# iamwinter/UMPR

Measured on AMD Instinct MI355X. Metric: training samples/sec, higher is better.
Workload: dtype f32

## Files before the change

include/umpr_hip.h:

```cpp
#ifndef UMPR_HIP_H
#define UMPR_HIP_H
#include <stddef.h>
#include <stdint.h>

#ifdef __cplusplus
extern "C" {
#endif

const char* umpr_version(void);
const char* umpr_last_error(void);
int umpr_device_info(int dev, char* name, int name_len, int* compute_units, size_t* hbm_bytes);

int umpr_gemm_f32(const float* A, long lda, int transA, const float* B, long ldb, int transB, float* C, long ldc,
                  int M, int N, int K, const float* bias, int bias_mode, int act, int accumulate, float alpha,
                  float* ws, size_t ws_bytes, void* stream);

int umpr_set_gemm_bf16(int on);

int umpr_set_conv_inference(int on);

int umpr_set_conv_pool_follows(int on);

long umpr_debug_wino_fix_count(void);

int umpr_debug_conv3x3_plan(int pass, int N, int Cin, int Cout, int H, int W, int inference, size_t* ws_bytes, size_t* v_bytes);
int umpr_debug_conv_bf16_plan(int pass, int N, int Cin, int Cout, int H, int W, long* out);

int umpr_debug_wino_pool_fold(const float* y, const float* g_pooled, const float* w, const float* x, float* unpooled, float* dx,
                              float* dw, float* db, int N, int Cin, int Cout, int H, int W, int f4, int fold, float* ws,
                              size_t ws_bytes, void* stream);

size_t umpr_embed_gru_bidir_ws_bytes(int N, int L, int E);
int umpr_embed_gru_bidir_fwd(const int64_t* ids, const float* emb, int E,
                             const float* w_ih_f, const float* w_hh_f, const float* b_ih_f, const float* b_hh_f,
                             const float* w_ih_r, const float* w_hh_r, const float* b_ih_r, const float* b_hh_r,
                             const int32_t* lengths, const int32_t* order, const int32_t* dst_row, int N, int L,
                             float* out, float* saved, float* ws, size_t ws_bytes, void* stream);
int umpr_embed_gru_bidir_bwd(const int64_t* ids, const float* emb, int E,
                             const float* w_hh_f, const float* w_hh_r,
                             const int32_t* lengths, const int32_t* order, const int32_t* dst_row, int N, int L,
                             const float* dout, const float* out, const float* saved,
                             float* dw_ih_f, float* dw_hh_f, float* db_ih_f, float* db_hh_f,
                             float* dw_ih_r, float* dw_hh_r, float* db_ih_r, float* db_hh_r,
                             float* ws, size_t ws_bytes, void* stream);

// ... 303 lines not shown
```

umpr_amd/_lib.py:

```python
from __future__ import annotations

import ctypes
import os
import threading

import torch

_HERE = os.path.dirname(os.path.abspath(__file__))
LIB_PATH = os.path.join(_HERE, "libumpr_hip.so")

_T = {"p": ctypes.c_void_p, "i": ctypes.c_int, "l": ctypes.c_long, "z": ctypes.c_size_t, "f": ctypes.c_float,
      "d": ctypes.c_double, "u": ctypes.c_uint64}

SIGNATURES = {
    "umpr_version": ("", "s"),
    "umpr_last_error": ("", "s"),
    "umpr_device_info": ("ipipp", "i"),
    "umpr_gemm_f32": ("pliplipliiipiiifpzp", "i"),
    "umpr_embed_gru_bidir_ws_bytes": ("iii", "z"),
    "umpr_embed_gru_bidir_fwd": ("ppipppppppppppiipppzp", "i"),
    "umpr_embed_gru_bidir_bwd": ("ppipppppiippppppppppppzp", "i"),
    "umpr_embed_gru_bidir_bwd_acc": ("ppipppppiipppppppppppipzp", "i"),
    "umpr_embed_gru_bidir_bwd_dx": ("ppipppppiipppppppppppipppipzp", "i"),
    "umpr_embed_grad_chunk": ("", "i"),
# ... 98 lines not shown
    "umpr_grad_norm": ("ppidfppzpp", "i"),
    "umpr_adam_step_clip": ("ppppldddddld" "pp", "i"),
    "umpr_adam_step_dev_clip": ("pppplddd" "ppp", "i"),
    "umpr_adam_step_groups": ("ppppldddddld" "pp" "ppp" "ii" "p", "i"),
    "umpr_grad_accumulate": ("pppiip", "i"),
    "umpr_ema_update": ("pppidip", "i"),
    "umpr_arena_swap": ("pppip", "i"),
    "umpr_debug_poison_lds": ("pp", "i"),
    "umpr_set_gemm_bf16": ("i", "i"),
    "umpr_set_conv_inference": ("i", "i"),
    "umpr_set_conv_pool_follows": ("i", "i"),
    "umpr_debug_wino_fix_count": ("", "l"),
    "umpr_debug_conv3x3_plan": ("iiiiiiipp", "i"),
    "umpr_debug_conv_bf16_plan": ("iiiiiip", "i"),
    "umpr_debug_wino_pool_fold": ("pppppppp" "iiiiiii" "pzp", "i"),
    "umpr_profile_enable": ("i", "i"),
    "umpr_profile_reset": ("", "i"),
    "umpr_profile_read": ("ippp", "i"),
}


class UmprHipError(RuntimeError):
    pass


class _Tls(threading.local):
    gemm_b16 = False


TLS = _Tls()
# ... 73 lines not shown
```

umpr_amd/csrc/api.hip:

```cpp
#include <math.h>
#include <stdarg.h>
#include <stdlib.h>

#include <vector>

#include "../../include/umpr_hip.h"
#include "umpr_common.h"
#include "umpr_internal.h"

static thread_local char g_err[512] = "";
void umpr_set_error(const char* fmt, ...) {
  va_list ap;
  va_start(ap, fmt);
  vsnprintf(g_err, sizeof(g_err), fmt, ap);
  va_end(ap);
}

namespace {
const bool g_fc_small = umpr_env_on("UMPR_FC_SMALL");
struct ProfRec { hipEvent_t e0, e1; int family; double work; };
bool g_prof_on = false;
std::vector<ProfRec> g_prof;
std::vector<ProfRec> g_prof_pool;
double g_prof_ms[UMPR_K_COUNT] = {0}, g_prof_work[UMPR_K_COUNT] = {0};
// ... 122 lines not shown
  UMPR_REQUIRE(!dx || (f4 && w), "debug_wino_pool_fold: the data gradient runs on the 4x4 tile and needs the weights");
  UMPR_REQUIRE(!dw || (x && (!f4 || ((H_ % 4) == 0 && (W % 4) == 0))), "debug_wino_pool_fold: the weight gradient on the 4x4 tile has no edge tiles");
  hipStream_t s = S(stream);
  ConvHints h;
  const float* g = g_pooled;
  if (fold) { h.pooled_dy = true; h.pool_y = y; }
  else {
    if (int rc = umpr_maxpool2_bwd_relu_impl(y, g_pooled, unpooled, (long)N * Cout, H_, W, s)) return rc;
    g = unpooled;
  }
  if (dx)
    if (int rc = umpr_wino_conv3x3(g, w, 1, nullptr, nullptr, dx, N, Cin, Cout, H_, W, 0, ws, ws_bytes / sizeof(float), true, h, s)) return rc;
  if (dw)
    if (int rc = umpr_wino_wgrad(g, x, dw, db, N, Cin, Cout, H_, W, 0, ws, ws_bytes / sizeof(float), f4 != 0, h, s)) return rc;
  return 0;
}

constexpr size_t kSlabs = 256;
namespace {
struct GruWs {
  float *gx, *wslab, *bslab;
  float* kslab; size_t kslab_bytes;
  float *stacked, *rows;
  float *wst, *bst;
  size_t bytes;
};
GruWs gru_ws(float* base, int N, int L, int pitch) {
  Carve c(base, sizeof(float));
  const size_t tiles = umpr_gru_tiles(N);
  GruWs w;
// ... 1011 lines not shown
```

umpr_amd/csrc/umpr_internal.h:

```cpp
#pragma once
#include <hip/hip_runtime.h>
#include <stdint.h>

struct UmprGemm {
  const float* A = nullptr; long lda = 0; bool transA = false;
  const float* B = nullptr; long ldb = 0; bool transB = false;
  float* C = nullptr; long ldc = 0;
  int M = 0, N = 0, K = 0;
  const int64_t* gatherA = nullptr;
  const int64_t* gatherB = nullptr;
  const float* bias = nullptr; int bias_mode = 0;
  int act = 0; bool accumulate = false; float alpha = 1.0f;
  int split_k = 1;
  float* ws = nullptr; size_t ws_bytes = 0;
  bool b16 = false;
  int winA_L = 0, winA_D = 1, winA_pad = 0;
  int winB_L = 0, winB_D = 1, winB_pad = 0;
};
int umpr_gemm(const UmprGemm& g, hipStream_t stream);
bool umpr_ambient_gemm_b16();

constexpr int D = 128, H = 64, G3 = 192, AT = 64;
bool umpr_merge_small();

// ... 52 lines not shown
  bool edge;
  size_t ws_floats;
  size_t v_floats;
};
ConvPlan umpr_conv3x3_plan(ConvPass pass, int N, int Cin, int Cout, int H, int W, bool inference);
size_t umpr_conv3x3_pack_floats(int N, int Cin, int Cout, int H, int W);
bool umpr_conv3x3_pool_fold_ok(int N, int Cin, int Cout, int H, int W);
int umpr_conv3x3_run(const float* x, const float* w, int transposed, const float* bias, const float* mask, float* y,
                     int N, int Cin, int Cout, int H, int W, int relu, float* wpack, size_t wpack_floats,
                     const ConvHints& hints, hipStream_t s);
struct WinoConvGeom { int planes, MT, S; long T, Tpad; bool edge; size_t v_floats, U, V, M, count, tie, floats; };
WinoConvGeom umpr_wino_conv_geom(int N, int C, int M, int H, int W, bool f4);
struct WinoWgradGeom { long T, Tpad; int MT, CT, Mpad, Cpad, stages, splits, stages_per_split, planes, bnc; size_t Gy, V, P, BP, floats; };
WinoWgradGeom umpr_wino_wgrad_geom(int N, int Cin, int Cout, int H, int W, bool f4);
long umpr_wino_last_fix_count();
int umpr_wino_wgrad(const float* dy, const float* x, float* dw, float* db, int N, int Cin, int Cout, int H, int W,
                    int accumulate, float* ws, size_t ws_floats, bool f4, const ConvHints& hints, hipStream_t s);
int umpr_wino_conv3x3(const float* x, const float* w, int transposed, const float* bias, const float* mask, float* y,
                      int N, int Cin, int Cout, int H, int W, int relu, float* ws, size_t ws_floats, bool f4,
                      const ConvHints& hints, hipStream_t s);
int umpr_conv3x3_flip_transpose(const float* w, float* wt, int Cout, int Cin, hipStream_t s);
size_t umpr_conv3x3_wgrad_ws_bytes(int N, int Cin, int Cout, int H, int W);
int umpr_conv3x3_wgrad(const float* gz, const float* x, float* dw, float* db, int N, int Cin, int Cout, int H, int W,
                       int accumulate, float* ws, size_t ws_bytes, const ConvHints& hints, hipStream_t s);
int umpr_maxpool2_fwd_impl(const float* x, float* y, long planes, int H, int W, hipStream_t s);
int umpr_maxpool2_bwd_relu_impl(const float* x, const float* gy, float* gx, long planes, int H, int W, hipStream_t s);

int umpr_wgrad_reduce(const float* slab, const float* bslab, int splits, int Cout, int Cin, float* dw, float* db,
                      int accumulate, hipStream_t s);

// ... 143 lines not shown
```

umpr_amd/csrc/winograd.hip:

```cpp
#include <type_traits>

#include "umpr_common.h"
#include "umpr_internal.h"

namespace {

constexpr int WK = 32;
constexpr int WBM = 128;
constexpr int WBN = 128;

__device__ __forceinline__ void pool_window_grad(const float2 a, const float2 b, const float gy, float2& ga, float2& gb) {
  int arg = 0;
  float m = a.x;
  if (a.y > m) { m = a.y; arg = 1; }
  if (b.x > m) { m = b.x; arg = 2; }
  if (b.y > m) { m = b.y; arg = 3; }
  const float g = m > 0.f ? gy : 0.f;
  ga = make_float2(arg == 0 ? g : 0.f, arg == 1 ? g : 0.f);
  gb = make_float2(arg == 2 ? g : 0.f, arg == 3 ? g : 0.f);
}
typedef float f32x4_t __attribute__((ext_vector_type(4)));
__device__ __forceinline__ float as_loaded(float v) { asm volatile("" : "+v"(v)); return v; }
__device__ __forceinline__ float4 as_loaded(const float4 v) {
  f32x4_t q = {v.x, v.y, v.z, v.w};
// ... 656 lines not shown
    for (int o = 32; o > 0; o >>= 1) acc += __shfl_xor(acc, o, 64);
    if (lane == 0) {
      float v = acc + (bias ? bias[m] : 0.f);
      if (relu) v = fmaxf(v, 0.f);
      y[idx] = v;
    }
  }
}

static long wino_tpad(long T) { return (T + WBN - 1) / WBN * WBN; }

struct WinoGemmParams {
  const float* U;
  const float* V;
  float* Mx;
  int MT, S, C;
  long Tpad;
  long TT;
  int Mpad;
  int planes;
};

typedef __attribute__((address_space(3))) void* lds_ptr_t;
template <int FOLD>
__global__ __launch_bounds__(256, 2) void wino_gemm_dma_kernel(WinoGemmParams p) {
  constexpr int SK = WK;
  constexpr int LD = 128;
  constexpr int TM = 2, TN = 2;
  constexpr int KS = SK / 2;
  constexpr int NP = SK / 8;
  constexpr int SFLUSH = 1;
  typedef typename std::conditional<FOLD == 2, double, float>::type tot_t;
  __shared__ __attribute__((aligned(1024))) float As[2][SK * LD];
  __shared__ __attribute__((aligned(1024))) float Bs[2][SK * LD];
  const int tid = threadIdx.x, lane = tid & 63;
  const int wave = __builtin_amdgcn_readfirstlane(tid >> 6);
  const int wm = wave >> 1, wn = wave & 1;
  const int l31 = lane & 31, half = lane >> 5;
  const long TT = p.TT;
  const int xcd = blockIdx.x & 7;
  const long qq = blockIdx.x >> 3;
  const int mt = (int)(qq % p.MT);
  const long bt = (qq / p.MT) * 8 + xcd;
  if (bt >= p.planes * TT) return;
  const int xi = (int)(bt / TT);
  const long t0 = (bt % TT) * WBN;
  const float* Ub = p.U + (((long)xi * p.MT + mt) * p.S) * (WK * WBM);
  const float* Vb = p.V + (long)xi * (p.S * WK) * p.Tpad + t0;
  const float* ga = Ub + wave * (NP * 256) + lane * 4;
  const float* gb = Vb + (long)(wave * (2 * NP) + half) * p.Tpad + l31 * 4;
  const long bstep = 2 * p.Tpad;
  const unsigned lds_a = (unsigned)(size_t)(lds_ptr_t)(&As[0][0]) + (unsigned)wave * (NP * 1024u);
  const unsigned lds_b = (unsigned)(size_t)(lds_ptr_t)(&Bs[0][0]) + (unsigned)wave * (NP * 1024u);
  auto glds = [&](const float* src, unsigned dst) {
    unsigned keep;
    asm volatile("s_mov_b32 %0, m0\n\ts_mov_b32 m0, %2\n\ts_nop 0\n\tglobal_load_lds_dwordx4 %1, off\n\ts_mov_b32 m0, %0"
                 : "=&s"(keep) : "v"(src), "s"(dst) : "memory");
  };
  auto dma = [&](int q, int sn, int nbuf) {
    if (q < NP) glds(ga + (long)sn * (SK * WBM) + q * 256, lds_a + (unsigned)nbuf * (SK * LD * 4u) + (unsigned)q * 1024u);
    else glds(gb + (long)sn * SK * p.Tpad + (q - NP) * bstep, lds_b + (unsigned)nbuf * (SK * LD * 4u) + (unsigned)(q - NP) * 1024u);
  };
  auto dma_wait = [&]() { asm volatile("s_waitcnt vmcnt(0)" ::: "memory"); };

  f32x16 acc[TM][TN];
  tot_t tot[TM][TN][16];
#pragma unroll
  for (int i = 0; i < TM; ++i)
#pragma unroll
    for (int j = 0; j < TN; ++j)
#pragma unroll
      for (int r = 0; r < 16; ++r) { acc[i][j][r] = 0.f; tot[i][j][r] = (tot_t)0; }

  const int ns = p.S * (WK / SK);
#pragma unroll
  for (int q = 0; q < 2 * NP; ++q) dma(q, 0, 0);
  dma_wait();
  __syncthreads();
  for (int s0 = 0; s0 < ns; s0 += SFLUSH) {
#pragma unroll
    for (int i = 0; i < TM; ++i)
#pragma unroll
      for (int j = 0; j < TN; ++j)
#pragma unroll
        for (int r = 0; r < 16; ++r) acc[i][j][r] = 0.f;
    const int s1 = min(ns, s0 + SFLUSH);
    for (int s = s0; s < s1; ++s) {
      const int cur = s & 1;
      const int sn = min(s + 1, ns - 1);
      const float* as = As[cur] + half * LD + wm * 64 + l31;
      const float* bs = Bs[cur] + half * LD + wn * 64 + l31;
      float a[2][TM], b[2][TN];
#pragma unroll
      for (int i = 0; i < TM; ++i) a[0][i] = as[i * 32];
#pragma unroll
      for (int j = 0; j < TN; ++j) b[0][j] = bs[j * 32];
#pragma unroll
      for (int kk = 0; kk < KS; ++kk) {
        const int cb = kk & 1, nb = cb ^ 1;
        const int k1 = kk + 1;
#pragma unroll
        for (int m = 0; m < TM * TN; ++m) {
          const int i = m / TN, j = m % TN;
          acc[i][j] = mfma32(a[cb][i], b[cb][j], acc[i][j]);
          if (m == 0 && k1 < KS) {
#pragma unroll
            for (int ii = 0; ii < TM; ++ii) a[nb][ii] = as[2 * k1 * LD + ii * 32];
          }
          if (m == 1 && k1 < KS) {
#pragma unroll
            for (int jj = 0; jj < TN; ++jj) b[nb][jj] = bs[2 * k1 * LD + jj * 32];
          }
          if (m == 3 && kk < 2 * NP) dma(kk, sn, cur ^ 1);
          __builtin_amdgcn_sched_barrier(0);
        }
      }
      dma_wait();
      __syncthreads();
    }
#pragma unroll
    for (int i = 0; i < TM; ++i)
#pragma unroll
      for (int j = 0; j < TN; ++j)
#pragma unroll
        for (int r = 0; r < 16; ++r) tot[i][j][r] += (tot_t)acc[i][j][r];
  }
  float* Mb = p.Mx + ((long)xi * p.Mpad + mt * WBM) * p.Tpad + t0;
#pragma unroll
  for (int i = 0; i < TM; ++i)
#pragma unroll
    for (int j = 0; j < TN; ++j)
#pragma unroll
      for (int r = 0; r < 16; ++r)
        Mb[(long)(wm * 64 + i * 32 + mfma_row(r, lane)) * p.Tpad + wn * 64 + j * 32 + l31] = (float)tot[i][j][r];
}

inline int nblk(long n, int cap) {
  long b = (n + 255) / 256;
  if (b > cap) b = cap;
  return (int)(b < 1 ? 1 : b);
}

}

static thread_local const unsigned int* t_last_fix_count = nullptr;
long umpr_wino_last_fix_count() {
  if (!t_last_fix_count) return -1;
  unsigned int v = 0;
  if (hipDeviceSynchronize() != hipSuccess || hipMemcpy(&v, t_last_fix_count, sizeof(v), hipMemcpyDeviceToHost) != hipSuccess) return -2;
  return (long)v;
}

WinoConvGeom umpr_wino_conv_geom(int N, int C, int M, int H, int W, bool f4) {
  WinoConvGeom g;
  g.planes = f4 ? 36 : 16; g.edge = f4 && ((H % 4) != 0 || (W % 4) != 0);
  g.T = f4 ? (long)N * ((H + 3) / 4) * ((W + 3) / 4) : (long)N * (H / 2) * (W / 2);
  g.Tpad = wino_tpad(g.T); g.MT = (M + WBM - 1) / WBM; g.S = (C + WK - 1) / WK;
  g.v_floats = (size_t)g.planes * g.S * WK * g.Tpad;
  g.U = 0; g.V = (size_t)g.planes * g.MT * WBM * g.S * WK; g.M = g.V + g.v_floats;
  g.count = g.M + (size_t)g.planes * g.MT * WBM * g.Tpad; g.tie = g.count + 16;
  g.floats = g.count + 64 + (f4 ? g.Tpad : 0);
  return g;
}


// ... 40 lines not shown
    UMPR_REQUIRE(f4 && transposed && hints.pool_y && !fix, "winograd: the pooled source needs a data gradient on the 4x4 tile");
    if (edge) wino4_input_kernel<true, false, true><<<nblk((long)S * WK * TT * WBN, 16384), 256, 0, s>>>(x, V, N, C, S * WK, H, W, Tpad, TT * WBN, wino4_consts(), nullptr, nullptr, hints.pool_y);
    else wino4_input_kernel<false, false, true><<<nblk((long)S * WK * TT * WBN, 16384), 256, 0, s>>>(x, V, N, C, S * WK, H, W, Tpad, TT * WBN, wino4_consts(), nullptr, nullptr, hints.pool_y);
  } else if (f4 && edge) {
    if (tie_bits) wino4_input_kernel<true, true><<<nblk((long)S * WK * TT * WBN, 16384), 256, 0, s>>>(x, V, N, C, S * WK, H, W, Tpad, TT * WBN, wino4_consts(), fx.count, tie_bits);
    else wino4_input_kernel<true, false><<<nblk((long)S * WK * TT * WBN, 16384), 256, 0, s>>>(x, V, N, C, S * WK, H, W, Tpad, TT * WBN, wino4_consts(), fx.count, nullptr);
  } else if (f4) {
    if (tie_bits) wino4_input_kernel<false, true><<<nblk((long)S * WK * TT * WBN, 16384), 256, 0, s>>>(x, V, N, C, S * WK, H, W, Tpad, TT * WBN, wino4_consts(), fx.count, tie_bits);
    else wino4_input_kernel<false, false><<<nblk((long)S * WK * TT * WBN, 16384), 256, 0, s>>>(x, V, N, C, S * WK, H, W, Tpad, TT * WBN, wino4_consts(), fx.count, nullptr);
  }
  else if ((W / 2) % 2 == 0)
    wino_input_pair_kernel<<<nblk((long)S * WK * TT * WBN / 2, 16384), 256, 0, s>>>(x, V, N, C, S * WK, H, W, Tpad, TT * WBN);
  else
    wino_input_kernel<<<nblk((long)S * WK * TT * WBN, 16384), 256, 0, s>>>(x, V, N, C, S * WK, H, W, Tpad, TT * WBN);
  UMPR_LAUNCH_CHECK("wino_input");
  WinoGemmParams p{U, V, Mx, MT, S, C, Tpad, TT, MT * WBM, planes};
  const long groups = (planes * TT + 7) / 8 * 8;
  {
    UmprProfScope prof(UMPR_K_WINO_GEMM, 2.0 * planes * (double)M * C * T, s);
    static const int fold = umpr_env_int("UMPR_WINO_FOLD", 1);
    if (fold == 2) wino_gemm_dma_kernel<2><<<(unsigned)(groups * MT), 256, 0, s>>>(p);
    else wino_gemm_dma_kernel<1><<<(unsigned)(groups * MT), 256, 0, s>>>(p);
  }
  UMPR_LAUNCH_CHECK("wino_gemm");
  if (f4 && fix) {
    if (edge) wino4_output_kernel<true, true><<<nblk((long)M * T, 16384), 256, 0, s>>>(Mx, bias, mask, y, N, M, H, W, Tpad, MT * WBM, relu, wino4_consts(), fx);
    else wino4_output_kernel<false, true><<<nblk((long)M * T, 16384), 256, 0, s>>>(Mx, bias, mask, y, N, M, H, W, Tpad, MT * WBM, relu, wino4_consts(), fx);
    UMPR_LAUNCH_CHECK("wino_output");
    wino_fixup_kernel<<<128, 256, 0, s>>>(x, w, bias, y, fx.list, fx.count, fx.cap, C, M, H, W, relu);
    UMPR_LAUNCH_CHECK("wino_fixup");
    t_last_fix_count = fx.count;
    return 0;
  }
  if (f4 && edge)
    wino4_output_kernel<true, false><<<nblk((long)M * T, 16384), 256, 0, s>>>(Mx, bias, mask, y, N, M, H, W, Tpad, MT * WBM, relu, wino4_consts(), fx);
  else if (f4)
    wino4_output_kernel<false, false><<<nblk((long)M * T, 16384), 256, 0, s>>>(Mx, bias, mask, y, N, M, H, W, Tpad, MT * WBM, relu, wino4_consts(), fx);
  else if ((W / 2) % 2 == 0)
    wino_output_pair_kernel<<<nblk((long)M * T / 2, 16384), 256, 0, s>>>(Mx, bias, mask, y, N, M, H, W, Tpad, MT * WBM, relu);
// ... 339 lines not shown

constexpr int WLDK = WK + 4;

template <int TN>
__global__ __launch_bounds__(256, 2) void wino_wgrad_gemm_kernel(WinoWgradParams p) {
  constexpr int LD = WLDK;
  constexpr int TM = 2;
  constexpr int BNC = 64 * TN;
  constexpr int NG = WK / 8;
  constexpr int SFLUSH = 4;
  __shared__ __attribute__((aligned(16))) float As[2][WBM * LD];
  __shared__ __attribute__((aligned(16))) float Bs[2][BNC * LD];
  const int tid = threadIdx.x, lane = tid & 63, wave = tid >> 6;
  const int wm = wave >> 1, wn = wave & 1;
  const int l31 = lane & 31, half = lane >> 5;
  long b = blockIdx.x;
  const int ct = (int)(b % p.CT); b /= p.CT;
  const int mt = (int)(b % p.MT); b /= p.MT;
  const int xi = (int)(b % p.planes);
  const int split = (int)(b / p.planes);
  const int s_begin = split * p.stages_per_split;
  const int s_end = min(p.stages, s_begin + p.stages_per_split);
  const int ns = s_end - s_begin;

  const int urow = tid >> 3, uq = tid & 7;
  const float* pa = p.Gy + ((long)xi * p.Mpad + mt * WBM + urow) * p.Tpad + (long)s_begin * WK + 4 * uq;
  const float* pb = p.V + ((long)xi * p.Cpad + ct * BNC + urow) * p.Tpad + (long)s_begin * WK + 4 * uq;
  const long rstep = 32 * p.Tpad;
  float* sa = &As[0][urow * LD + 4 * uq];
  float* sb = &Bs[0][urow * LD + 4 * uq];
  float4 ra0, ra1, ra2, ra3, rb0, rb1, rb2, rb3;
  auto lda = [&](int v, int s) { return *reinterpret_cast<const float4*>(pa + (long)s * WK + v * rstep); };
  auto ldb = [&](int v, int s) { return *reinterpret_cast<const float4*>(pb + (long)s * WK + v * rstep); };
  auto sta = [&](int v, int buf, const float4& r) { *reinterpret_cast<float4*>(sa + buf * (WBM * LD) + 32 * v * LD) = r; };
  auto stb = [&](int v, int buf, const float4& r) { *reinterpret_cast<float4*>(sb + buf * (BNC * LD) + 32 * v * LD) = r; };
// ... 9 lines not shown
      case 7: if (TN == 2) rb3 = ldb(3, sn); break;
      case 8: sta(0, nbuf, ra0); break;
      case 9: sta(1, nbuf, ra1); break;
      case 10: sta(2, nbuf, ra2); break;
      case 11: sta(3, nbuf, ra3); break;
      case 12: stb(0, nbuf, rb0); break;
      case 13: stb(1, nbuf, rb1); break;
      case 14: if (TN == 2) stb(2, nbuf, rb2); break;
      default: if (TN == 2) stb(3, nbuf, rb3); break;
    }
  };
  auto comp = [](const float4& v, int e) { return e == 0 ? v.x : e == 1 ? v.y : e == 2 ? v.z : v.w; };

  f32x16 acc[TM][TN], tot[TM][TN];
#pragma unroll
  for (int i = 0; i < TM; ++i)
#pragma unroll
    for (int j = 0; j < TN; ++j)
#pragma unroll
      for (int r = 0; r < 16; ++r) { acc[i][j][r] = 0.f; tot[i][j][r] = 0.f; }

#pragma unroll
  for (int q = 0; q < 16; ++q) piece(q, 0, 0);
  __syncthreads();
  for (int s0 = 0; s0 < ns; s0 += SFLUSH) {
#pragma unroll
    for (int i = 0; i < TM; ++i)
#pragma unroll
      for (int j = 0; j < TN; ++j)
#pragma unroll
        for (int r = 0; r < 16; ++r) acc[i][j][r] = 0.f;
    const int s1 = min(ns, s0 + SFLUSH);
    for (int s = s0; s < s1; ++s) {
      const int cur = s & 1;
      const int sn = min(s + 1, ns - 1);
      const float* as = As[cur] + (wm * 64 + l31) * LD + 4 * half;
      const float* bs = Bs[cur] + (wn * 32 * TN + l31) * LD + 4 * half;
      float4 a[2][TM], bq[2][TN];
// ... 18 lines not shown
#pragma unroll
              for (int jj = 0; jj < TN; ++jj) bq[nb][jj] = *reinterpret_cast<const float4*>(bs + jj * 32 * LD + 8 * (g + 1));
            }
            if (m == TM * TN - 1) piece(4 * g + e, sn, cur ^ 1);
            __builtin_amdgcn_sched_barrier(0);
          }
        }
      }
      __syncthreads();
    }
#pragma unroll
    for (int i = 0; i < TM; ++i)
#pragma unroll
      for (int j = 0; j < TN; ++j) tot[i][j] += acc[i][j];
  }
  float* Pb = p.P + ((((long)split * p.planes + xi) * p.Mpad + mt * WBM) * p.Cpad) + ct * BNC;
#pragma unroll
  for (int i = 0; i < TM; ++i)
#pragma unroll
    for (int j = 0; j < TN; ++j)
#pragma unroll
      for (int r = 0; r < 16; ++r)
        Pb[(long)(wm * 64 + i * 32 + mfma_row(r, lane)) * p.Cpad + wn * 32 * TN + j * 32 + l31] = tot[i][j][r];
}

__global__ void wino_wgrad_finish_kernel(const float* __restrict__ P, int splits, int Mch, int C, int Mpad, int Cpad,
                                         float* __restrict__ dw, int accumulate) {
  const long total = (long)Mch * C;
  const long per = (long)Mpad * Cpad;
  for (long i = blockIdx.x * (long)blockDim.x + threadIdx.x; i < total; i += (long)gridDim.x * blockDim.x) {
    const int c = (int)(i % C);
    const int m = (int)(i / C);
    float v[4][4];
#pragma unroll
    for (int a = 0; a < 16; ++a) {
      float acc = 0.f;
      for (int sp = 0; sp < splits; ++sp) acc += P[((long)sp * 16 + a) * per + (long)m * Cpad + c];
      v[a >> 2][a & 3] = acc;
// ... 43 lines not shown
      if (eff > best) best = eff;
    }
    for (int sp = 1; sp <= hi; ++sp) {
      const long wgs = (long)tiles * sp;
      if (wgs < 512) continue;
      if ((double)wgs / (double)((wgs + 511) / 512 * 512) >= best - 0.03) { splits = sp; break; }
    }
  }
  if (splits > max_splits) splits = max_splits;
  if (splits < 1) splits = 1;
  g.stages_per_split = (g.stages + splits - 1) / splits;
  g.splits = (g.stages + g.stages_per_split - 1) / g.stages_per_split;
  g.Gy = 0; g.V = (size_t)g.planes * g.Mpad * g.Tpad; g.P = g.V + (size_t)g.planes * g.Cpad * g.Tpad;
  g.BP = g.P + (size_t)g.planes * g.splits * g.Mpad * g.Cpad; g.floats = g.BP + (size_t)g.Mpad * (g.Tpad / 64) + 64;
  return g;
}

int umpr_wino_wgrad(const float* dy, const float* x, float* dw, float* db, int N, int Cin, int Cout, int H, int W,
                    int accumulate, float* ws, size_t ws_floats, bool f4, const ConvHints& hints, hipStream_t s) {
  const WinoWgradGeom g = umpr_wino_wgrad_geom(N, Cin, Cout, H, W, f4);
  UMPR_REQUIRE(ws_floats >= g.floats, "winograd wgrad: workspace too small");
  UMPR_REQUIRE((H % 2) == 0 && (W % 2) == 0, "winograd wgrad: odd map %dx%d", H, W);
  float *Gy = ws + g.Gy, *V = ws + g.V, *P = ws + g.P, *BP = ws + g.BP;
  const bool edge = f4 && ((H % 4) != 0 || (W % 4) != 0);
  static const bool bias_fuse = umpr_env_on("UMPR_WINO_BIAS_FUSE");
  const bool fused_bias = db && f4 && !edge && bias_fuse && (g.Tpad % 64) == 0;
  const bool pooled = hints.pooled_dy;
  const float* py = hints.pool_y;
  if (pooled) UMPR_REQUIRE(py && !edge, "winograd wgrad: the pooled source needs the layer's output and whole tiles");
  if (f4 && edge)
// ... 13 lines not shown
  }
  UMPR_LAUNCH_CHECK("wino_dy");
  if (hints.v_slot) {
    UMPR_REQUIRE(f4 && !edge && hints.v_slot_floats == (size_t)g.planes * g.Cpad * g.Tpad,
                 "winograd wgrad: the V slot does not match this layer (%d -> %d at %dx%d)", Cin, Cout, H, W);
    V = hints.v_slot;
  } else if (f4 && edge)
    wino4_input_kernel<true, false><<<nblk((long)g.Cpad * g.Tpad, 16384), 256, 0, s>>>(x, V, N, Cin, g.Cpad, H, W, g.Tpad, g.Tpad, wino4_consts(), nullptr, nullptr);
  else if (f4)
    wino4_input_kernel<false, false><<<nblk((long)g.Cpad * g.Tpad, 16384), 256, 0, s>>>(x, V, N, Cin, g.Cpad, H, W, g.Tpad, g.Tpad, wino4_consts(), nullptr, nullptr);
  else if ((W / 2) % 2 == 0)
    wino_input_pair_kernel<<<nblk((long)g.Cpad * g.Tpad / 2, 16384), 256, 0, s>>>(x, V, N, Cin, g.Cpad, H, W, g.Tpad, g.Tpad);
  else
    wino_input_kernel<<<nblk((long)g.Cpad * g.Tpad, 16384), 256, 0, s>>>(x, V, N, Cin, g.Cpad, H, W, g.Tpad, g.Tpad);
  UMPR_LAUNCH_CHECK("wino_input(wgrad)");
  WinoWgradParams p{Gy, V, P, g.MT, g.CT, g.Mpad, g.Cpad, g.Tpad, g.stages, g.stages_per_split, g.planes};
  {
    UmprProfScope prof(UMPR_K_WINO_WGRAD_GEMM, 2.0 * g.planes * (double)Cout * Cin * g.T, s);
    if (g.bnc == 64) wino_wgrad_gemm_kernel<1><<<(unsigned)(g.planes * g.MT * g.CT * g.splits), 256, 0, s>>>(p);
    else wino_wgrad_gemm_kernel<2><<<(unsigned)(g.planes * g.MT * g.CT * g.splits), 256, 0, s>>>(p);
  }
  UMPR_LAUNCH_CHECK("wino_wgrad_gemm");
  if (f4)
    wino4_wgrad_finish_kernel<<<(unsigned)((long)Cout * ((Cin + 63) / 64)), 256, 0, s>>>(P, g.splits, Cout, Cin, g.Mpad, g.Cpad, dw,
                                                                                     accumulate, wino4_consts());
  else if (g.splits >= 8)
    wino_wgrad_finish_wide_kernel<<<(unsigned)((long)Cout * ((Cin + 63) / 64)), 256, 0, s>>>(P, g.splits, Cout, Cin, g.Mpad, g.Cpad,
                                                                                         dw, accumulate);
  else
    wino_wgrad_finish_kernel<<<nblk((long)Cout * Cin, 4096), 256, 0, s>>>(P, g.splits, Cout, Cin, g.Mpad, g.Cpad, dw, accumulate);
  UMPR_LAUNCH_CHECK("wino_wgrad_finish");
  if (fused_bias) {
    wino_bias_sum_waves_kernel<<<(unsigned)((Cout + 3) / 4), 256, 0, s>>>(BP, db, Cout, g.Tpad / 64, accumulate);
    UMPR_LAUNCH_CHECK("wino_bias_sum_waves");
  } else if (db) {
    UMPR_REQUIRE((size_t)N * Cout <= (size_t)g.splits * g.planes * g.Mpad * g.Cpad && ((long)H * W) % 4 == 0,
                 "winograd wgrad: bias-gradient scratch");
// ... 9 lines not shown
```

Before: 2173.

## Restructure Winograd GEMM main loop with double accumulators and cheaper addressing

Rewrites the Winograd forward GEMM kernel's stage loop. Each SK-step stage is now an unrolled parity-templated stage, with two accumulator sets so the fold of the previous stage's partial sums into the running total is spread across the MFMA issue slots. LDS offsets are advanced incrementally, and the global-to-LDS DMA uses a scalar base plus vector offset. Index math moves to 32-bit unsigned, and the output stores use a strength-reduced row pointer, with the same store pattern applied to the wgrad GEMM kernel. The wgrad kernel also overlaps its initial DMA with accumulator zeroing. The gains depend on register pressure, since the extra accumulator set may lower occupancy. Debug entry points and launch wrappers with 32-bit range checks are added.

```diff
diff --git a/include/umpr_hip.h b/include/umpr_hip.h
--- a/include/umpr_hip.h
+++ b/include/umpr_hip.h
@@ -29,6 +29,11 @@
 int umpr_debug_wino_pool_fold(const float* y, const float* g_pooled, const float* w, const float* x, float* unpooled, float* dx,
                               float* dw, float* db, int N, int Cin, int Cout, int H, int W, int f4, int fold, float* ws,
                               size_t ws_bytes, void* stream);
+
+int umpr_debug_wino_gemm(const float* U, const float* V, float* M, int planes, int MT, int S, long TT, long Tpad, int fold,
+                         void* stream);
+int umpr_debug_wino_wgrad_gemm(const float* Gy, const float* V, float* P, int planes, int MT, int CT, int TN, long Tpad,
+                               int stages_per_split, void* stream);
 
 size_t umpr_embed_gru_bidir_ws_bytes(int N, int L, int E);
 int umpr_embed_gru_bidir_fwd(const int64_t* ids, const float* emb, int E,
diff --git a/umpr_amd/_lib.py b/umpr_amd/_lib.py
--- a/umpr_amd/_lib.py
+++ b/umpr_amd/_lib.py
@@ -136,6 +136,8 @@
     "umpr_debug_conv3x3_plan": ("iiiiiiipp", "i"),
     "umpr_debug_conv_bf16_plan": ("iiiiiip", "i"),
     "umpr_debug_wino_pool_fold": ("pppppppp" "iiiiiii" "pzp", "i"),
+    "umpr_debug_wino_gemm": ("ppp" "iiillip", "i"),
+    "umpr_debug_wino_wgrad_gemm": ("ppp" "iiiilip", "i"),
     "umpr_profile_enable": ("i", "i"),
     "umpr_profile_reset": ("", "i"),
     "umpr_profile_read": ("ippp", "i"),
diff --git a/umpr_amd/csrc/api.hip b/umpr_amd/csrc/api.hip
--- a/umpr_amd/csrc/api.hip
+++ b/umpr_amd/csrc/api.hip
@@ -160,6 +160,14 @@
   if (dw)
     if (int rc = umpr_wino_wgrad(g, x, dw, db, N, Cin, Cout, H_, W, 0, ws, ws_bytes / sizeof(float), f4 != 0, h, s)) return rc;
   return 0;
+}
+int umpr_debug_wino_gemm(const float* U, const float* V, float* M, int planes, int MT, int S_, long TT, long Tpad, int fold,
+                         void* stream) {
+  return umpr_wino_gemm_launch(U, V, M, planes, MT, S_, TT, Tpad, fold, S(stream));
+}
+int umpr_debug_wino_wgrad_gemm(const float* Gy, const float* V, float* P, int planes, int MT, int CT, int TN, long Tpad,
+                               int stages_per_split, void* stream) {
+  return umpr_wino_wgrad_gemm_launch(Gy, V, P, planes, MT, CT, TN, Tpad, stages_per_split, S(stream));
 }
 
 constexpr size_t kSlabs = 256;
diff --git a/umpr_amd/csrc/umpr_internal.h b/umpr_amd/csrc/umpr_internal.h
--- a/umpr_amd/csrc/umpr_internal.h
+++ b/umpr_amd/csrc/umpr_internal.h
@@ -90,6 +90,10 @@
 struct WinoWgradGeom { long T, Tpad; int MT, CT, Mpad, Cpad, stages, splits, stages_per_split, planes, bnc; size_t Gy, V, P, BP, floats; };
 WinoWgradGeom umpr_wino_wgrad_geom(int N, int Cin, int Cout, int H, int W, bool f4);
 long umpr_wino_last_fix_count();
+int umpr_wino_gemm_launch(const float* U, const float* V, float* Mx, int planes, int MT, int S, long TT, long Tpad, int fold,
+                          hipStream_t s);
+int umpr_wino_wgrad_gemm_launch(const float* Gy, const float* V, float* P, int planes, int MT, int CT, int TN, long Tpad,
+                                int stages_per_split, hipStream_t s);
 int umpr_wino_wgrad(const float* dy, const float* x, float* dw, float* db, int N, int Cin, int Cout, int H, int W,
                     int accumulate, float* ws, size_t ws_floats, bool f4, const ConvHints& hints, hipStream_t s);
 int umpr_wino_conv3x3(const float* x, const float* w, int transposed, const float* bias, const float* mask, float* y,
diff --git a/umpr_amd/csrc/winograd.hip b/umpr_amd/csrc/winograd.hip
--- a/umpr_amd/csrc/winograd.hip
+++ b/umpr_amd/csrc/winograd.hip
@@ -694,11 +694,11 @@
   const float* U;
   const float* V;
   float* Mx;
-  int MT, S, C;
+  int MT, S;
   long Tpad;
-  long TT;
+  int TT;
+  int PT;
   int Mpad;
-  int planes;
 };
 
 typedef __attribute__((address_space(3))) void* lds_ptr_t;
@@ -709,110 +709,159 @@
   constexpr int TM = 2, TN = 2;
   constexpr int KS = SK / 2;
   constexpr int NP = SK / 8;
-  constexpr int SFLUSH = 1;
+  constexpr int NSET = FOLD == 1 ? 2 : 1;
+  constexpr int FOLD_K0 = 2;
   typedef typename std::conditional<FOLD == 2, double, float>::type tot_t;
-  __shared__ __attribute__((aligned(1024))) float As[2][SK * LD];
-  __shared__ __attribute__((aligned(1024))) float Bs[2][SK * LD];
+  __shared__ __attribute__((aligned(1024))) float Ls[4][SK * LD];
   const int tid = threadIdx.x, lane = tid & 63;
   const int wave = __builtin_amdgcn_readfirstlane(tid >> 6);
   const int wm = wave >> 1, wn = wave & 1;
   const int l31 = lane & 31, half = lane >> 5;
-  const long TT = p.TT;
-  const int xcd = blockIdx.x & 7;
-  const long qq = blockIdx.x >> 3;
-  const int mt = (int)(qq % p.MT);
-  const long bt = (qq / p.MT) * 8 + xcd;
-  if (bt >= p.planes * TT) return;
-  const int xi = (int)(bt / TT);
-  const long t0 = (bt % TT) * WBN;
-  const float* Ub = p.U + (((long)xi * p.MT + mt) * p.S) * (WK * WBM);
-  const float* Vb = p.V + (long)xi * (p.S * WK) * p.Tpad + t0;
-  const float* ga = Ub + wave * (NP * 256) + lane * 4;
-  const float* gb = Vb + (long)(wave * (2 * NP) + half) * p.Tpad + l31 * 4;
+  const unsigned xcd = blockIdx.x & 7u, qq = blockIdx.x >> 3;
+  const unsigned mt = qq % (unsigned)p.MT;
+  const unsigned bt = (qq / (unsigned)p.MT) * 8u + xcd;
+  if (bt >= (unsigned)p.PT) return;
+  const unsigned xi = bt / (unsigned)p.TT;
+  const unsigned t0 = (bt % (unsigned)p.TT) * WBN;
+  const int ns = p.S;
+  const float* an = p.U + (((long)xi * p.MT + mt) * p.S) * (WK * WBM) + wave * (NP * 256);
+  const float* bn = p.V + (long)xi * (p.S * WK) * p.Tpad + t0 + (long)(wave * (2 * NP)) * p.Tpad;
+  const unsigned va = (unsigned)lane * 16u;
+  const unsigned vb = ((unsigned)half * (unsigned)p.Tpad + (unsigned)l31 * 4u) * 4u;
   const long bstep = 2 * p.Tpad;
-  const unsigned lds_a = (unsigned)(size_t)(lds_ptr_t)(&As[0][0]) + (unsigned)wave * (NP * 1024u);
-  const unsigned lds_b = (unsigned)(size_t)(lds_ptr_t)(&Bs[0][0]) + (unsigned)wave * (NP * 1024u);
-  auto glds = [&](const float* src, unsigned dst) {
+  const unsigned lds_a = (unsigned)(size_t)(lds_ptr_t)(&Ls[0][0]) + (unsigned)wave * (NP * 1024u);
+  const unsigned lds_b = (unsigned)(size_t)(lds_ptr_t)(&Ls[2][0]) + (unsigned)wave * (NP * 1024u);
+  auto glds = [&](const float* base, unsigned voff, unsigned dst) {
     unsigned keep;
-    asm volatile("s_mov_b32 %0, m0\n\ts_mov_b32 m0, %2\n\ts_nop 0\n\tglobal_load_lds_dwordx4 %1, off\n\ts_mov_b32 m0, %0"
-                 : "=&s"(keep) : "v"(src), "s"(dst) : "memory");
+    asm volatile("s_mov_b32 %0, m0\n\ts_mov_b32 m0, %3\n\ts_nop 0\n\tglobal_load_lds_dwordx4 %1, %2\n\ts_mov_b32 m0, %0"
+                 : "=&s"(keep) : "v"(voff), "s"(base), "s"(dst) : "memory");
   };
-  auto dma = [&](int q, int sn, int nbuf) {
-    if (q < NP) glds(ga + (long)sn * (SK * WBM) + q * 256, lds_a + (unsigned)nbuf * (SK * LD * 4u) + (unsigned)q * 1024u);
-    else glds(gb + (long)sn * SK * p.Tpad + (q - NP) * bstep, lds_b + (unsigned)nbuf * (SK * LD * 4u) + (unsigned)(q - NP) * 1024u);
+  auto dma = [&](int q, int nbuf) {
+    if (q < NP) glds(an + q * 256, va, lds_a + (unsigned)nbuf * (SK * LD * 4u) + (unsigned)q * 1024u);
+    else glds(bn + (q - NP) * bstep, vb, lds_b + (unsigned)nbuf * (SK * LD * 4u) + (unsigned)(q - NP) * 1024u);
   };
   auto dma_wait = [&]() { asm volatile("s_waitcnt vmcnt(0)" ::: "memory"); };
 
-  f32x16 acc[TM][TN];
+#pragma unroll
+  for (int q = 0; q < 2 * NP; ++q) dma(q, 0);
+  int more = ns - 1;
+  if (more > 0) { an += SK * WBM; bn += (long)SK * p.Tpad; }
+  --more;
+
+  f32x16 acc[NSET][TM][TN];
   tot_t tot[TM][TN][16];
 #pragma unroll
   for (int i = 0; i < TM; ++i)
 #pragma unroll
     for (int j = 0; j < TN; ++j)
 #pragma unroll
-      for (int r = 0; r < 16; ++r) { acc[i][j][r] = 0.f; tot[i][j][r] = (tot_t)0; }
-
-  const int ns = p.S * (WK / SK);
-#pragma unroll
-  for (int q = 0; q < 2 * NP; ++q) dma(q, 0, 0);
+      for (int r = 0; r < 16; ++r) {
+        float z0, z1;
+        asm volatile("v_mov_b32 %0, 0\n\tv_mov_b32 %1, 0" : "=v"(z0), "=v"(z1));
+        acc[NSET - 1][i][j][r] = z0; tot[i][j][r] = (tot_t)z1;
+      }
+
+  unsigned oa = (unsigned)(half * LD + wm * 64 + l31) * 4u, ob = (unsigned)(2 * SK * LD + half * LD + wn * 64 + l31) * 4u;
+  auto frag_a = [&](int ii) { return reinterpret_cast<const float*>(reinterpret_cast<const char*>(&Ls[0][0]) + oa)[ii * 32]; };
+  auto frag_b = [&](int jj) { return reinterpret_cast<const float*>(reinterpret_cast<const char*>(&Ls[0][0]) + ob)[jj * 32]; };
+  float a[2][TM], b[2][TN];
   dma_wait();
   __syncthreads();
-  for (int s0 = 0; s0 < ns; s0 += SFLUSH) {
-#pragma unroll
-    for (int i = 0; i < TM; ++i)
-#pragma unroll
-      for (int j = 0; j < TN; ++j)
-#pragma unroll
-        for (int r = 0; r < 16; ++r) acc[i][j][r] = 0.f;
-    const int s1 = min(ns, s0 + SFLUSH);
-    for (int s = s0; s < s1; ++s) {
-      const int cur = s & 1;
-      const int sn = min(s + 1, ns - 1);
-      const float* as = As[cur] + half * LD + wm * 64 + l31;
-      const float* bs = Bs[cur] + half * LD + wn * 64 + l31;
-      float a[2][TM], b[2][TN];
-#pragma unroll
-      for (int i = 0; i < TM; ++i) a[0][i] = as[i * 32];
-#pragma unroll
-      for (int j = 0; j < TN; ++j) b[0][j] = bs[j * 32];
-#pragma unroll
-      for (int kk = 0; kk < KS; ++kk) {
-        const int cb = kk & 1, nb = cb ^ 1;
-        const int k1 = kk + 1;
-#pragma unroll
-        for (int m = 0; m < TM * TN; ++m) {
-          const int i = m / TN, j = m % TN;
-          acc[i][j] = mfma32(a[cb][i], b[cb][j], acc[i][j]);
-          if (m == 0 && k1 < KS) {
-#pragma unroll
-            for (int ii = 0; ii < TM; ++ii) a[nb][ii] = as[2 * k1 * LD + ii * 32];
-          }
-          if (m == 1 && k1 < KS) {
-#pragma unroll
-            for (int jj = 0; jj < TN; ++jj) b[nb][jj] = bs[2 * k1 * LD + jj * 32];
-          }
-          if (m == 3 && kk < 2 * NP) dma(kk, sn, cur ^ 1);
-          __builtin_amdgcn_sched_barrier(0);
+#pragma unroll
+  for (int i = 0; i < TM; ++i) a[0][i] = frag_a(i);
+#pragma unroll
+  for (int j = 0; j < TN; ++j) b[0][j] = frag_b(j);
+
+  auto stage = [&](auto parity) {
+    constexpr int X = decltype(parity)::value;
+    constexpr int A = X % NSET, F = (X ^ 1) % NSET;
+    constexpr unsigned STEP = 2 * LD * 4, BUF = SK * LD * 4;
+    constexpr unsigned CROSS = X == 0 ? BUF - (KS - 1) * STEP : 0u - BUF - (KS - 1) * STEP;
+#pragma unroll
+    for (int kk = 0; kk < KS; ++kk) {
+      const int cb = kk & 1, nb = cb ^ 1;
+      const int k1 = kk + 1;
+      if (kk == KS - 1) {
+        dma_wait();
+        __syncthreads();
+      }
+#pragma unroll
+      for (int m = 0; m < TM * TN; ++m) {
+        const int i = m / TN, j = m % TN;
+        if (kk == 0) {
+          const f32x16 zero = {0.f, 0.f, 0.f, 0.f, 0.f, 0.f, 0.f, 0.f, 0.f, 0.f, 0.f, 0.f, 0.f, 0.f, 0.f, 0.f};
+          acc[A][i][j] = mfma32(a[cb][i], b[cb][j], zero);
+        } else {
+          acc[A][i][j] = mfma32(a[cb][i], b[cb][j], acc[A][i][j]);
         }
-      }
-      dma_wait();
-      __syncthreads();
-    }
-#pragma unroll
-    for (int i = 0; i < TM; ++i)
-#pragma unroll
-      for (int j = 0; j < TN; ++j)
-#pragma unroll
-        for (int r = 0; r < 16; ++r) tot[i][j][r] += (tot_t)acc[i][j][r];
-  }
-  float* Mb = p.Mx + ((long)xi * p.Mpad + mt * WBM) * p.Tpad + t0;
+        if (m == 0) {
+          oa += k1 < KS ? STEP : CROSS;
+          asm volatile("" : "+v"(oa));
+#pragma unroll
+          for (int ii = 0; ii < TM; ++ii) a[nb][ii] = frag_a(ii);
+        }
+        if (m == 1) {
+          ob += k1 < KS ? STEP : CROSS;
+          asm volatile("" : "+v"(ob));
+#pragma unroll
+          for (int jj = 0; jj < TN; ++jj) b[nb][jj] = frag_b(jj);
+        }
+        if (m == 3 && kk < 2 * NP) dma(kk, X ^ 1);
+        if (NSET == 2 && kk >= FOLD_K0 && kk < FOLD_K0 + 8) {
+          const int e = (kk - FOLD_K0) * (TM * TN) + m;
+          const int fi = (e / 8) / TN, fj = (e / 8) % TN, r = 2 * (e % 8);
+          tot[fi][fj][r] += (tot_t)acc[F][fi][fj][r];
+          tot[fi][fj][r + 1] += (tot_t)acc[F][fi][fj][r + 1];
+        }
+        __builtin_amdgcn_sched_barrier(0);
+      }
+    }
+    if (NSET == 1) {
+#pragma unroll
+      for (int i = 0; i < TM; ++i)
+#pragma unroll
+        for (int j = 0; j < TN; ++j)
+#pragma unroll
+          for (int r = 0; r < 16; ++r) tot[i][j][r] += (tot_t)acc[0][i][j][r];
+    }
+    if (more > 0) { an += SK * WBM; bn += (long)SK * p.Tpad; }
+    --more;
+  };
+
+  int s = 0;
+  for (; s + 1 < ns; s += 2) {
+    stage(std::integral_constant<int, 0>{});
+    stage(std::integral_constant<int, 1>{});
+  }
+  if (s < ns) stage(std::integral_constant<int, 0>{});
+  if (NSET == 2) {
+    if (ns & 1) {
+#pragma unroll
+      for (int i = 0; i < TM; ++i)
+#pragma unroll
+        for (int j = 0; j < TN; ++j)
+#pragma unroll
+          for (int r = 0; r < 16; ++r) tot[i][j][r] += (tot_t)acc[0][i][j][r];
+    } else {
+#pragma unroll
+      for (int i = 0; i < TM; ++i)
+#pragma unroll
+        for (int j = 0; j < TN; ++j)
+#pragma unroll
+          for (int r = 0; r < 16; ++r) tot[i][j][r] += (tot_t)acc[NSET - 1][i][j][r];
+    }
+  }
+  float* Mb = p.Mx + ((long)xi * p.Mpad + (long)mt * WBM + wm * 64) * p.Tpad + t0 + wn * 64;
+  const unsigned tp = (unsigned)p.Tpad;
+  unsigned row = (unsigned)(4 * half) * tp + (unsigned)l31;
 #pragma unroll
   for (int i = 0; i < TM; ++i)
 #pragma unroll
-    for (int j = 0; j < TN; ++j)
-#pragma unroll
-      for (int r = 0; r < 16; ++r)
-        Mb[(long)(wm * 64 + i * 32 + mfma_row(r, lane)) * p.Tpad + wn * 64 + j * 32 + l31] = (float)tot[i][j][r];
+    for (int r = 0; r < 16; ++r) {
+#pragma unroll
+      for (int j = 0; j < TN; ++j) (Mb + j * 32)[row] = (float)tot[i][j][r];
+      row += (r & 3) == 3 ? 5u * tp : tp;
+    }
 }
 
 inline int nblk(long n, int cap) {
@@ -829,6 +878,20 @@
   unsigned int v = 0;
   if (hipDeviceSynchronize() != hipSuccess || hipMemcpy(&v, t_last_fix_count, sizeof(v), hipMemcpyDeviceToHost) != hipSuccess) return -2;
   return (long)v;
+}
+
+int umpr_wino_gemm_launch(const float* U, const float* V, float* Mx, int planes, int MT, int S, long TT, long Tpad, int fold,
+                          hipStream_t s) {
+  UMPR_REQUIRE(U && V && Mx && planes > 0 && MT > 0 && S > 0 && TT > 0 && Tpad >= TT * WBN && (Tpad % 4) == 0 &&
+               (fold == 1 || fold == 2), "wino_gemm: bad arguments");
+  const long groups = (planes * TT + 7) / 8 * 8;
+  UMPR_REQUIRE(groups * MT < 0x7fffffffL && Tpad < (1L << 23), "wino_gemm: %ld workgroups / rows of %ld tiles do not fit 32 bits",
+               groups * MT, Tpad);
+  WinoGemmParams p{U, V, Mx, MT, S, Tpad, (int)TT, (int)(planes * TT), MT * WBM};
+  if (fold == 2) wino_gemm_dma_kernel<2><<<(unsigned)(groups * MT), 256, 0, s>>>(p);
+  else wino_gemm_dma_kernel<1><<<(unsigned)(groups * MT), 256, 0, s>>>(p);
+  UMPR_LAUNCH_CHECK("wino_gemm");
+  return 0;
 }
 
 WinoConvGeom umpr_wino_conv_geom(int N, int C, int M, int H, int W, bool f4) {
@@ -899,15 +962,11 @@
   else
     wino_input_kernel<<<nblk((long)S * WK * TT * WBN, 16384), 256, 0, s>>>(x, V, N, C, S * WK, H, W, Tpad, TT * WBN);
   UMPR_LAUNCH_CHECK("wino_input");
-  WinoGemmParams p{U, V, Mx, MT, S, C, Tpad, TT, MT * WBM, planes};
-  const long groups = (planes * TT + 7) / 8 * 8;
   {
     UmprProfScope prof(UMPR_K_WINO_GEMM, 2.0 * planes * (double)M * C * T, s);
     static const int fold = umpr_env_int("UMPR_WINO_FOLD", 1);
-    if (fold == 2) wino_gemm_dma_kernel<2><<<(unsigned)(groups * MT), 256, 0, s>>>(p);
-    else wino_gemm_dma_kernel<1><<<(unsigned)(groups * MT), 256, 0, s>>>(p);
-  }
-  UMPR_LAUNCH_CHECK("wino_gemm");
+    if (int rc = umpr_wino_gemm_launch(U, V, Mx, planes, MT, S, TT, Tpad, fold, s)) return rc;
+  }
   if (f4 && fix) {
     if (edge) wino4_output_kernel<true, true><<<nblk((long)M * T, 16384), 256, 0, s>>>(Mx, bias, mask, y, N, M, H, W, Tpad, MT * WBM, relu, wino4_consts(), fx);
     else wino4_output_kernel<false, true><<<nblk((long)M * T, 16384), 256, 0, s>>>(Mx, bias, mask, y, N, M, H, W, Tpad, MT * WBM, relu, wino4_consts(), fx);
@@ -1277,11 +1336,11 @@
   const int tid = threadIdx.x, lane = tid & 63, wave = tid >> 6;
   const int wm = wave >> 1, wn = wave & 1;
   const int l31 = lane & 31, half = lane >> 5;
-  long b = blockIdx.x;
-  const int ct = (int)(b % p.CT); b /= p.CT;
-  const int mt = (int)(b % p.MT); b /= p.MT;
-  const int xi = (int)(b % p.planes);
-  const int split = (int)(b / p.planes);
+  unsigned b = blockIdx.x;
+  const int ct = (int)(b % (unsigned)p.CT); b /= (unsigned)p.CT;
+  const int mt = (int)(b % (unsigned)p.MT); b /= (unsigned)p.MT;
+  const int xi = (int)(b % (unsigned)p.planes);
+  const int split = (int)(b / (unsigned)p.planes);
   const int s_begin = split * p.stages_per_split;
   const int s_end = min(p.stages, s_begin + p.stages_per_split);
   const int ns = s_end - s_begin;
@@ -1321,14 +1380,19 @@
 
   f32x16 acc[TM][TN], tot[TM][TN];
 #pragma unroll
+  for (int q = 0; q < 8; ++q) piece(q, 0, 0);
+#pragma unroll
   for (int i = 0; i < TM; ++i)
 #pragma unroll
     for (int j = 0; j < TN; ++j)
 #pragma unroll
-      for (int r = 0; r < 16; ++r) { acc[i][j][r] = 0.f; tot[i][j][r] = 0.f; }
-
-#pragma unroll
-  for (int q = 0; q < 16; ++q) piece(q, 0, 0);
+      for (int r = 0; r < 16; ++r) {
+        float z;
+        asm volatile("v_mov_b32 %0, 0" : "=v"(z));
+        tot[i][j][r] = z;
+      }
+#pragma unroll
+  for (int q = 8; q < 16; ++q) piece(q, 0, 0);
   __syncthreads();
   for (int s0 = 0; s0 < ns; s0 += SFLUSH) {
 #pragma unroll
@@ -1377,14 +1441,17 @@
 #pragma unroll
       for (int j = 0; j < TN; ++j) tot[i][j] += acc[i][j];
   }
-  float* Pb = p.P + ((((long)split * p.planes + xi) * p.Mpad + mt * WBM) * p.Cpad) + ct * BNC;
+  float* Pb = p.P + ((((long)split * p.planes + xi) * p.Mpad + mt * WBM + wm * 64) * p.Cpad) + ct * BNC + wn * 32 * TN;
+  const unsigned cp = (unsigned)p.Cpad;
+  unsigned row = (unsigned)(4 * half) * cp + (unsigned)l31;
 #pragma unroll
   for (int i = 0; i < TM; ++i)
 #pragma unroll
-    for (int j = 0; j < TN; ++j)
-#pragma unroll
-      for (int r = 0; r < 16; ++r)
-        Pb[(long)(wm * 64 + i * 32 + mfma_row(r, lane)) * p.Cpad + wn * 32 * TN + j * 32 + l31] = tot[i][j][r];
+    for (int r = 0; r < 16; ++r) {
+#pragma unroll
+      for (int j = 0; j < TN; ++j) (Pb + j * 32)[row] = tot[i][j][r];
+      row += (r & 3) == 3 ? 5u * cp : cp;
+    }
 }
 
 __global__ void wino_wgrad_finish_kernel(const float* __restrict__ P, int splits, int Mch, int C, int Mpad, int Cpad,
@@ -1458,6 +1525,21 @@
   g.Gy = 0; g.V = (size_t)g.planes * g.Mpad * g.Tpad; g.P = g.V + (size_t)g.planes * g.Cpad * g.Tpad;
   g.BP = g.P + (size_t)g.planes * g.splits * g.Mpad * g.Cpad; g.floats = g.BP + (size_t)g.Mpad * (g.Tpad / 64) + 64;
   return g;
+}
+
+int umpr_wino_wgrad_gemm_launch(const float* Gy, const float* V, float* P, int planes, int MT, int CT, int TN, long Tpad,
+                                int stages_per_split, hipStream_t s) {
+  UMPR_REQUIRE(Gy && V && P && planes > 0 && MT > 0 && CT > 0 && (TN == 1 || TN == 2) && Tpad > 0 && (Tpad % WK) == 0 &&
+               Tpad / WK < 0x7fffffffL && stages_per_split > 0, "wino_wgrad_gemm: bad arguments");
+  const int stages = (int)(Tpad / WK);
+  const int splits = (stages + stages_per_split - 1) / stages_per_split;
+  const long wgs = (long)planes * MT * CT * splits;
+  UMPR_REQUIRE(wgs < 0x7fffffffL && CT < (1 << 16), "wino_wgrad_gemm: %ld workgroups / %d channel tiles do not fit 32 bits", wgs, CT);
+  WinoWgradParams p{Gy, V, P, MT, CT, MT * WBM, CT * 64 * TN, Tpad, stages, stages_per_split, planes};
+  if (TN == 1) wino_wgrad_gemm_kernel<1><<<(unsigned)wgs, 256, 0, s>>>(p);
+  else wino_wgrad_gemm_kernel<2><<<(unsigned)wgs, 256, 0, s>>>(p);
+  UMPR_LAUNCH_CHECK("wino_wgrad_gemm");
+  return 0;
 }
 
 int umpr_wino_wgrad(const float* dy, const float* x, float* dw, float* db, int N, int Cin, int Cout, int H, int W,
@@ -1501,13 +1583,10 @@
   else
     wino_input_kernel<<<nblk((long)g.Cpad * g.Tpad, 16384), 256, 0, s>>>(x, V, N, Cin, g.Cpad, H, W, g.Tpad, g.Tpad);
   UMPR_LAUNCH_CHECK("wino_input(wgrad)");
-  WinoWgradParams p{Gy, V, P, g.MT, g.CT, g.Mpad, g.Cpad, g.Tpad, g.stages, g.stages_per_split, g.planes};
   {
     UmprProfScope prof(UMPR_K_WINO_WGRAD_GEMM, 2.0 * g.planes * (double)Cout * Cin * g.T, s);
-    if (g.bnc == 64) wino_wgrad_gemm_kernel<1><<<(unsigned)(g.planes * g.MT * g.CT * g.splits), 256, 0, s>>>(p);
-    else wino_wgrad_gemm_kernel<2><<<(unsigned)(g.planes * g.MT * g.CT * g.splits), 256, 0, s>>>(p);
-  }
-  UMPR_LAUNCH_CHECK("wino_wgrad_gemm");
+    if (int rc = umpr_wino_wgrad_gemm_launch(Gy, V, P, g.planes, g.MT, g.CT, g.bnc / 64, g.Tpad, g.stages_per_split, s)) return rc;
+  }
   if (f4)
     wino4_wgrad_finish_kernel<<<(unsigned)((long)Cout * ((Cin + 63) / 64)), 256, 0, s>>>(P, g.splits, Cout, Cin, g.Mpad, g.Cpad, dw,
                                                                                      accumulate, wino4_consts());
```

After: 2171. Within noise of the previous version (-0.1%).
